# efirdc/Segmentation-Pipeline

Hardware: AMD Instinct MI355X
Metric: 3D patches/sec (128³, 4ch) train+infer at 1/2/4/8 MI355X; Dice vs CPU ref (higher is better)
Workload: dtype f32 (tensors, results and accumulation; the products of the 3x3x3 convolutions with >= 8 input channels run as six bf16 MFMAs on an EXACT three-way bf16 split of both f32 operands -- error vs f64 equal to the f32 MFMA kernels', profiles/r04_f32x3_accuracy.txt; the same step on v_mfma_f32_32x32x2_f32

## Files before the change

### include/m355seg.h

```cpp
#ifndef M355SEG_H
#define M355SEG_H

#include <stddef.h>
#include <stdint.h>

#ifdef __cplusplus
extern "C" {
#endif

#define M355_ABI_VERSION 3

enum {
  M355_OK = 0,
  M355_EINVALID_ARG = -1,
  M355_EUNSUPPORTED = -2,
  M355_ELAUNCH = -3,
  M355_EWORKSPACE = -4
};

enum { M355_F32 = 0 };

enum { M355_COMPUTE_F32 = 0, M355_COMPUTE_BF16 = 1, M355_COMPUTE_F16 = 2, M355_COMPUTE_F32X3 = 3 };

enum { M355_ACT_NONE = 0, M355_ACT_RELU = 1, M355_ACT_LEAKY_RELU = 2, M355_ACT_ELU = 3, M355_ACT_GELU = 4,
// ... 68 lines not shown

int m355_conv3d_launch_plan(int32_t entry, const m355_conv3d_desc* d, const int64_t* batch_strides, const uint64_t* pointers,
                            size_t workspace_bytes, int64_t* out12);

size_t m355_conv3d_bwd_data_workspace(const m355_conv3d_desc* d);
int m355_conv3d_bwd_data(const m355_conv3d_desc* d, const float* dy, const float* w,
                         float* dx, void* workspace, size_t workspace_bytes, void* stream);

size_t m355_conv3d_bwd_weight_workspace(const m355_conv3d_desc* d);
int m355_conv3d_bwd_weight(const m355_conv3d_desc* d, const float* x, const float* dy,
                           float* dw, float* dbias,
                           void* workspace, size_t workspace_bytes, void* stream);

size_t m355_conv_transpose3d_workspace(const m355_conv3d_desc* d);
int m355_conv_transpose3d_fwd(const m355_conv3d_desc* d, const float* x, const float* w,
                              const float* bias, float* y,
                              void* workspace, size_t workspace_bytes, void* stream);
int m355_conv_transpose3d_bwd_data(const m355_conv3d_desc* d, const float* dy, const float* w,
                                   float* dx, void* workspace, size_t workspace_bytes,
                                   void* stream);
int m355_conv_transpose3d_bwd_weight(const m355_conv3d_desc* d, const float* x, const float* dy,
                                     float* dw, float* dbias,
                                     void* workspace, size_t workspace_bytes, void* stream);

int m355_conv_transpose3d_plan(const m355_conv3d_desc* d, int32_t which, const void* y_side, int32_t* out4);

int32_t m355_conv_transpose3d_x3_bwd_supported(const m355_conv3d_desc* d, const void* y_side);
size_t m355_conv_transpose3d_x3_bwd_workspace(const m355_conv3d_desc* d);
int m355_conv_transpose3d_x3_bwd_plan(const m355_conv3d_desc* d, int32_t which, const void* y_side, int32_t* out4);
int m355_conv_transpose3d_bwd_data_x3(const m355_conv3d_desc* d, const float* dy, const float* w, float* dx,
                                      void* workspace, size_t workspace_bytes, void* stream);
int m355_conv_transpose3d_bwd_weight_x3(const m355_conv3d_desc* d, const float* x, const float* dy, float* dw, float* dbias,
                                        void* workspace, size_t workspace_bytes, void* stream);

int m355_conv_transpose3d_fwd_h16(const m355_conv3d_desc* d, const void* x16, int64_t x16_batch_stride,
                                  const float* w, const float* bias, void* y16, int64_t y16_batch_stride,
                                  int32_t compute, void* stream);

typedef struct m355_norm_desc {
  int32_t N, C;
  int64_t S;
  int32_t groups;
  int32_t act;
  float eps;
  float act_slope;
  int64_t x_batch_stride;
  int64_t y_batch_stride;
  int64_t add_batch_stride;
} m355_norm_desc;

int64_t m355_norm_num_stats(const m355_norm_desc* d);
size_t m355_norm_workspace(const m355_norm_desc* d);

int m355_norm_plan(const m355_norm_desc* d, int32_t which, int32_t* out4);

int m355_norm_stats(const m355_norm_desc* d, const float* x, float* mean, float* rstd,
                    float* running_mean, float* running_var, float momentum,
                    void* workspace, size_t workspace_bytes, void* stream);
int m355_norm_stats_from_partials(const m355_norm_desc* d, const float* stat_partials, int64_t slots,
                                  float* mean, float* rstd, float* running_mean, float* running_var,
                                  float momentum, void* workspace, size_t workspace_bytes, void* stream);
int m355_norm_stats_from_running(const m355_norm_desc* d, const float* running_mean,
                                 const float* running_var, float* mean, float* rstd,
                                 void* stream);
int m355_norm_act_fwd(const m355_norm_desc* d, const float* x, const float* mean,
                      const float* rstd, const float* gamma, const float* beta,
// ... 526 lines not shown
```

### segmentation-pipeline_amd/_lib.py

```python
import ctypes as C
import os

_HERE = os.path.dirname(os.path.abspath(__file__))
LIB_PATH = os.environ.get("M355_LIB_PATH") or os.path.join(_HERE, "libm355seg.so")

M355_OK = 0
M355_EUNSUPPORTED = -2
ACT_NONE, ACT_RELU, ACT_LEAKY_RELU = 0, 1, 2
ACT_ELU, ACT_GELU, ACT_GELU_TANH, ACT_SILU = 3, 4, 5, 6
COMPUTE_F32, COMPUTE_BF16, COMPUTE_F16, COMPUTE_F32X3 = 0, 1, 2, 3
CONV_W_PACKED, CONV_SOFTMAX, CONV_SIGMOID = 1, 2, 4


class ConvDesc(C.Structure):
    _fields_ = [
        ("N", C.c_int32), ("Cin", C.c_int32), ("Cout", C.c_int32),
        ("D", C.c_int32), ("H", C.c_int32), ("W", C.c_int32),
        ("k", C.c_int32), ("stride", C.c_int32), ("pad", C.c_int32), ("out_pad", C.c_int32),
        ("x_batch_stride", C.c_int64), ("y_batch_stride", C.c_int64),
        ("compute", C.c_int32), ("flags", C.c_int32),
    ]


class PackItem(C.Structure):
# ... 156 lines not shown
    "m355_norm_act_bwd_c8": (C.c_int, [_ND, _P, _i64, _P, _i64, _P, _i64, _i32, _i32, _i32, _P, _P, _P, _P, _P, _i64, _P, _P,
                                       C.c_int, _f32, _i32, _P, _sz, _P]),
    "m355_norm_act_bwd_c8_reduce": (C.c_int, [_ND, _P, _i64, _P, _i64, _P, _i64, _i32, _i32, _i32, _P, _P, _P, _P, _P, _P,
                                              C.c_int, _P, _f32, _P, _i32, _P, _sz, _P]),
    "m355_norm_act_bwd_c8_apply": (C.c_int, [_ND, _P, _i64, _P, _i64, _P, _i64, _i32, _i32, _i32, _P, _P, _P, _P, _P, _P, _i64,
                                             _i32, _P]),
    "m355_avgpool3d_2x_bwd_h16": (C.c_int, [_P, _P, _P, _i32, _i32, _i32, _i32, _i32, _i64, _i64, _i64, _i32, _P]),
    "m355_upsample_trilinear2x_fwd_h16": (C.c_int, [_P, _P, _i32, _i32, _i32, _i32, _i32, _i64, _i64, _i32, _P]),
    "m355_upsample_trilinear2x_bwd_h16": (C.c_int, [_P, _P, _i32, _i32, _i32, _i32, _i32, _i64, _i64, _i32, _P]),
    "m355_act16_channel_scale": (C.c_int, [_P, _P, _P, _i32, _i32, _i64, _i64, _i64, _i32, _P]),
    "m355_space_to_depth2_h16": (C.c_int, [_P, _P, _i32, _i32, _i32, _i32, _i32, _i64, _i64, _i32, _P]),
    "m355_depth_to_space2_h16": (C.c_int, [_P, _P, _i32, _i32, _i32, _i32, _i32, _i64, _i64, _i32, _P]),
    "m355_conv_transpose3d_h16_bwd_supported": (_i32, [_CD]),
    "m355_conv_transpose3d_h16_bwd_workspace": (_sz, [_CD]),
    "m355_conv_transpose3d_bwd_data_h16": (C.c_int, [_CD, _P, _i64, _P, _P, _i64, _i32, _P]),
    "m355_conv_transpose3d_bwd_weight_h16": (C.c_int, [_CD, _P, _i64, _P, _i64, _P, _P, _f32, _i32, _P, _sz, _P]),
    "m355_conv3d_plan": (C.c_int, [_CD, _i32, C.POINTER(C.c_int32)]),
    "m355_conv3d_launch_plan": (C.c_int, [_i32, _CD, C.POINTER(_i64), C.POINTER(C.c_uint64), _sz, C.POINTER(_i64)]),
    "m355_conv3d_bwd_data_workspace": (_sz, [_CD]),
    "m355_conv3d_bwd_data": (C.c_int, [_CD, _P, _P, _P, _P, _sz, _P]),
    "m355_conv3d_bwd_weight_workspace": (_sz, [_CD]),
    "m355_conv3d_bwd_weight": (C.c_int, [_CD, _P, _P, _P, _P, _P, _sz, _P]),
    "m355_conv_transpose3d_workspace": (_sz, [_CD]),
    "m355_conv_transpose3d_plan": (C.c_int, [_CD, _i32, _P, C.POINTER(C.c_int32)]),
    "m355_conv_transpose3d_fwd": (C.c_int, [_CD, _P, _P, _P, _P, _P, _sz, _P]),
    "m355_conv_transpose3d_bwd_data": (C.c_int, [_CD, _P, _P, _P, _P, _sz, _P]),
    "m355_conv_transpose3d_bwd_weight": (C.c_int, [_CD, _P, _P, _P, _P, _P, _sz, _P]),
    "m355_conv_transpose3d_fwd_h16": (C.c_int, [_CD, _P, _i64, _P, _P, _P, _i64, _i32, _P]),
    "m355_conv_transpose3d_x3_bwd_supported": (_i32, [_CD, _P]),
    "m355_conv_transpose3d_x3_bwd_workspace": (_sz, [_CD]),
    "m355_conv_transpose3d_x3_bwd_plan": (C.c_int, [_CD, _i32, _P, C.POINTER(C.c_int32)]),
    "m355_conv_transpose3d_bwd_data_x3": (C.c_int, [_CD, _P, _P, _P, _P, _sz, _P]),
    "m355_conv_transpose3d_bwd_weight_x3": (C.c_int, [_CD, _P, _P, _P, _P, _P, _sz, _P]),
    "m355_norm_num_stats": (_i64, [_ND]),
    "m355_norm_workspace": (_sz, [_ND]),
    "m355_norm_plan": (C.c_int, [_ND, _i32, C.POINTER(C.c_int32)]),
    "m355_norm_stats": (C.c_int, [_ND, _P, _P, _P, _P, _P, _f32, _P, _sz, _P]),
    "m355_norm_stats_from_partials": (C.c_int, [_ND, _P, _i64, _P, _P, _P, _P, _f32, _P, _sz, _P]),
    "m355_norm_stats_from_running": (C.c_int, [_ND, _P, _P, _P, _P, _P]),
    "m355_norm_act_fwd": (C.c_int, [_ND, _P, _P, _P, _P, _P, _P, _P, _P]),
    "m355_norm_act_pool_fwd": (C.c_int, [_ND, _P, _P, _P, _P, _P, _P, _P, _i64, _i32, _i32, _i32, _P]),
    "m355_norm_act_bwd": (C.c_int, [_ND, _P, _P, _P, _P, _P, _P, _P, _P, _P, C.c_int, _P, _sz, _P]),
    "m355_norm_act_bwd_pool": (C.c_int, [_ND, _P, _P, _i64, _P, _i64, _i32, _i32, _i32, _P, _P, _P, _P, _P, _P, _P, C.c_int,
                                         _P, _sz, _P]),
    "m355_norm_sums": (C.c_int, [_ND, _P, _P, _i64, _P, _P, _sz, _P]),
    "m355_norm_stats_from_sums": (C.c_int, [_ND, _P, _P, _P, _P, _P, _f32, _P]),
    "m355_norm_act_bwd_reduce": (C.c_int, [_ND, _P, _P, _P, _P, _P, _P, _P, _P, C.c_int, _P, _P, _P, _sz, _P]),
    "m355_norm_act_bwd_apply": (C.c_int, [_ND, _P, _P, _P, _P, _P, _P, _P, _P, _P, _i64, _i32, _P]),
    "m355_norm_act_bwd_h16": (C.c_int, [_ND, _P, _P, _P, _P, _P, _P, _P, _P, _P, C.c_int, _P, _i64, _i32, _P, _sz, _P]),
    "m355_resample_plan": (C.c_int, [_i32, _i32, _i32, _i32, _i32, _i32, C.POINTER(_i64), C.POINTER(C.c_uint64), _i32,
                                     C.POINTER(_i64)]),
    "m355_avgpool3d_2x_fwd": (C.c_int, [_P, _P, _i32, _i32, _i32, _i32, _i32, _i64, _i64, _P]),
    "m355_avgpool3d_2x_bwd": (C.c_int, [_P, _P, _i32, _i32, _i32, _i32, _i32, _i64, _i64, _P]),
    "m355_avgpool3d_2x_bwd_add": (C.c_int, [_P, _P, _P, _i32, _i32, _i32, _i32, _i32, _i64, _i64, _i64, _P]),
    "m355_maxpool3d_2x_fwd": (C.c_int, [_P, _P, _P, _i32, _i32, _i32, _i32, _i32, _i64, _i64, _P]),
    "m355_maxpool3d_2x_bwd": (C.c_int, [_P, _P, _P, _P, _i32, _i32, _i32, _i32, _i32, _i64, _i64, _i64, _P]),
    "m355_maxpool3d_2x_fwd_h16": (C.c_int, [_P, _P, _P, _i32, _i32, _i32, _i32, _i32, _i64, _i64, _i32, _P]),
    "m355_maxpool3d_2x_bwd_h16": (C.c_int, [_P, _P, _P, _P, _i32, _i32, _i32, _i32, _i32, _i64, _i64, _i64, _i32, _P]),
    "m355_upsample_trilinear2x_fwd": (C.c_int, [_P, _P, _i32, _i32, _i32, _i32, _i32, _i64, _i64, _P]),
    "m355_upsample_trilinear2x_bwd": (C.c_int, [_P, _P, _i32, _i32, _i32, _i32, _i32, _i64, _i64, _P]),
    "m355_upsample_nearest2x_fwd": (C.c_int, [_P, _P, _i32, _i32, _i32, _i32, _i32, _i64, _i64, _P]),
    "m355_upsample_nearest2x_bwd": (C.c_int, [_P, _P, _i32, _i32, _i32, _i32, _i32, _i64, _i64, _P]),
    "m355_upsample_trilinear2x_hp_fwd": (C.c_int, [_P, _P, _i32, _i32, _i32, _i32, _i32, _i64, _i64, _P]),
    "m355_upsample_trilinear2x_hp_bwd": (C.c_int, [_P, _P, _i32, _i32, _i32, _i32, _i32, _i64, _i64, _P]),
    "m355_upsample_nearest2x_fwd_h16": (C.c_int, [_P, _P, _i32, _i32, _i32, _i32, _i32, _i64, _i64, _i32, _P]),
    "m355_upsample_nearest2x_bwd_h16": (C.c_int, [_P, _P, _i32, _i32, _i32, _i32, _i32, _i64, _i64, _i32, _P]),
# ... 215 lines not shown
```

### segmentation-pipeline_amd/csrc/abi.cpp

```cpp
#include "common.hpp"
#include <map>
#include <mutex>
#include <tuple>
#include <utility>

namespace m355 {
static thread_local char g_err[512] = "";
void set_error(const char* fmt, ...) {
  va_list ap;
  va_start(ap, fmt);
  vsnprintf(g_err, sizeof(g_err), fmt, ap);
  va_end(ap);
}

static int env_int(const char* name, int dflt) {
  const char* v = getenv(name);
  if (!v || !*v) return dflt;
  return atoi(v);
}
static Tuning read_tuning() {
  Tuning t;
  t.conv_ntw = env_int("M355_CONV_NTW", 0);
  t.conv_ksplit = env_int("M355_CONV_KSPLIT", 0);
  t.conv_slots = env_int("M355_CONV_SLOTS", 0);
  t.conv_persistent = env_int("M355_CONV_PERSISTENT", 1);
  t.no_small = env_int("M355_NO_SMALL", 0);
  t.smallcout_valu = env_int("M355_SMALLCOUT_VALU", 1);
  t.f32x3 = env_int("M355_F32X3", 1);
  t.f32x3_bww = env_int("M355_F32X3_BWW", 1);
  t.f32x3_edge = env_int("M355_F32X3_EDGE", 0);
  t.f32x3_convt = env_int("M355_F32X3_CONVT", 1);
  t.f32x3_convt_bwd = env_int("M355_F32X3_CONVT_BWD", 1);
  t.bww_nsplit = env_int("M355_BWW_NSPLIT", 0);
  t.bww_gen = env_int("M355_BWW_GEN", 2);
  t.bww_queue = env_int("M355_BWW_QUEUE", 1);
  t.h16_persistent = env_int("M355_H16_PERSISTENT", 1);
  t.tile16 = env_int("M355_TILE16", 1);
  t.convt_h16 = env_int("M355_CONVT_H16", 1);
  t.h16_w8 = env_int("M355_H16_W8", 1);
  t.h16_oneshot = env_int("M355_H16_ONESHOT", 1);
  t.h16_xcd = env_int("M355_H16_XCD", 1);
  t.conv_cube = env_int("M355_CONV_CUBE", 3);
  t.h16_order = env_int("M355_H16_ORDER", 3);
  t.fuse_softmax = env_int("M355_FUSE_SOFTMAX", 1);
  t.convt_wgs = env_int("M355_CONVT_WGS", 0);
  t.h16_stagger = env_int("M355_H16_STAGGER", 2);
  return t;
}
static Tuning g_tuning = read_tuning();
const Tuning& tuning() { return g_tuning; }

int num_cus() {
  static int cache[64] = {0};
  int dev = 0;
  if (hipGetDevice(&dev) != hipSuccess || dev < 0 || dev >= 64) {
    (void)hipGetLastError();
    return 256;
  }
  if (cache[dev] == 0) {
    int n = 0;
    if (hipDeviceGetAttribute(&n, hipDeviceAttributeMultiprocessorCount, dev) != hipSuccess || n <= 0) {
      (void)hipGetLastError();
      n = 256;
    }
    cache[dev] = n;
// ... 86 lines not shown
```

### segmentation-pipeline_amd/csrc/common.hpp

```cpp
#pragma once
#include <hip/hip_runtime.h>
#include <stdint.h>
#include <stdio.h>
#include <stdarg.h>
#include <stdlib.h>
#include <algorithm>
#include "../../include/m355seg.h"

namespace m355 {

void set_error(const char* fmt, ...);

static inline int64_t ceil_div(int64_t a, int64_t b) { return (a + b - 1) / b; }
static inline int64_t round_up(int64_t a, int64_t b) { return ceil_div(a, b) * b; }

static inline int check_launch(const char* what) {
  hipError_t e = hipGetLastError();
  if (e != hipSuccess) {
    set_error("%s: launch failed: %s", what, hipGetErrorString(e));
    return M355_ELAUNCH;
  }
  return M355_OK;
}

// ... 24 lines not shown
    const uint32_t o = (uint32_t)__shfl_up((int)v, off, 64);
    if (lane >= off) v += o;
  }
  return v;
}

template <typename T, int NT, bool BCAST = false>
__device__ __forceinline__ T block_sum(T v, T* scratch) {
  v = wave_sum(v);
  const int lane = threadIdx.x & 63, w = threadIdx.x >> 6;
  __syncthreads();
  if (lane == 0) scratch[w] = v;
  __syncthreads();
  T r = T(0);
  if (BCAST || threadIdx.x == 0) {
#pragma unroll
    for (int i = 0; i < NT / 64; ++i) r += scratch[i];
  }
  return r;
}

__device__ __forceinline__ float sigmoid_f32(float v) { return 1.f / (1.f + expf(-v)); }

struct Tuning {
  int conv_ntw = 0, conv_ksplit = 0, conv_slots = 0, conv_persistent = 1;
  int no_small = 0, smallcout_valu = 1, bww_nsplit = 0, bww_gen = 2, bww_queue = 1, h16_persistent = 1, tile16 = 1, convt_h16 = 1, h16_w8 = 1, h16_oneshot = 1, h16_xcd = 1;
  int conv_cube = 3, h16_order = 3;
  int fuse_softmax = 1;
  int f32x3 = 1;
  int f32x3_bww = 1;
  int f32x3_edge = 0;
  int f32x3_convt = 1;
  int f32x3_convt_bwd = 1;
  int convt_wgs = 0;
  int h16_stagger = 2;
};
const Tuning& tuning();

static inline int64_t dense_or(int64_t stride, int64_t dense) { return stride ? stride : dense; }

int num_cus();

int* queue_state(hipStream_t st);
int* overflow_flag();

}
```

### segmentation-pipeline_amd/csrc/conv3d_common.hpp

```cpp
#pragma once
#include "common.hpp"
#include "h16.hpp"
#include "conv3d_route.hpp"

namespace m355 {


__device__ __forceinline__ int opaque(int v) {
  asm volatile("" : "+v"(v));
  return v;
}

__device__ __forceinline__ void queue_leave(int* __restrict__ counter) {
  if (threadIdx.x == 0) {
    if (atomicAdd(counter + 8, 1) == (int)gridDim.x - 1) {
#pragma unroll
      for (int r = 0; r < 9; ++r) counter[r] = 0;
    }
  }
}

template <int NTW, int GX>
struct FwdTile {
  static constexpr int GY = 32 / GX;
// ... 122 lines not shown
        }
      }
      if (ok) {
#pragma unroll
        for (int r = 0; r < 4; ++r)
          if (ob + r < Cout) dst[base + (int64_t)r * DHW] = v[r];
      }
    }
  if (stat) {
#pragma unroll
    for (int r = 0; r < 4; ++r) {
#pragma unroll
      for (int off = 8; off >= 1; off >>= 1) {
        s1[r] += __shfl_xor(s1[r], off, 64);
        s2[r] += __shfl_xor(s2[r], off, 64);
      }
    }
    if ((lane & 15) == 0) {
#pragma unroll
      for (int r = 0; r < 4; ++r)
        if (ob + r < Cout) {
          stat[(int64_t)(ob + r) * 2] = s1[r];
          stat[(int64_t)(ob + r) * 2 + 1] = s2[r];
        }
    }
  }
}

int convt_fwd_x3_nvt(int Cin);
void launch_convt_fwd_x3(int nvt, dim3 grid, const float* x, const float* w, const float* bias, float* y, int Cin, int Cout,
                         int D, int H, int W, int64_t xbs, int64_t ybs, int mt_per_wg, hipStream_t st);
void launch_convt_bww_x3(int mt, dim3 grid, const float* x, const float* dy, float* dw, float* dbias, float* slab, double* bslab,
                         int N, int Cin, int Cout, int D, int H, int W, int64_t xbs, int64_t ybs, hipStream_t st);

enum class ConvtKind {
  Direct,
  MfmaF32,
  X3,
  C8,
  H16,
  Unsupported
};
struct ConvtRoute {
  ConvtKind kind;
  int nvt;
  int mt;
  int mt_per_wg;
  int ks_n, ng;
  dim3 grid;
  size_t lds;
  int split, o_per_split;
  size_t slab_bytes;
  size_t dbias_offset, dbias_bytes;
  size_t workspace_bytes;
  int32_t plan_code[4];
};
ConvtRoute route_convt(const m355_conv3d_desc* d, int which, bool y_side_ok);
ConvtRoute route_convt_c8(const m355_conv3d_desc* d, int which);

struct ConvCall {
  const m355_conv3d_desc* d;
  const float* in;
  const void* in16;
  const float* w;
  const float* bias;
  const float* add;
// ... 86 lines not shown
```

### segmentation-pipeline_amd/csrc/conv3d_f32x3.hip

```cpp
#include "conv3d_common.hpp"

namespace m355 {

typedef __bf16 bf16x8 __attribute__((ext_vector_type(8)));
typedef unsigned u32x4 __attribute__((ext_vector_type(4)));

constexpr int X3_PAIRS = 14;
constexpr int X3_QUADS = 7;
__host__ __device__ constexpr int x3_pair_tap(int pair, int half) {
  return pair < 9 ? pair * 3 + half : (pair < 12 ? (pair - 9) * 9 + half * 3 + 2 : (pair == 12 ? half * 9 + 8 : 26));
}

__device__ __forceinline__ void x3_split(float v, unsigned& hi, unsigned& mid, unsigned& lo) {
  const unsigned u = __float_as_uint(v);
  hi = u & 0xffff0000u;
  const float r1 = (u & 0x7f800000u) == 0x7f800000u ? 0.f : v - __uint_as_float(hi);
  mid = __float_as_uint(r1) & 0xffff0000u;
  lo = __float_as_uint(r1 - __uint_as_float(mid));
}
__device__ __forceinline__ unsigned x3_pack(unsigned a, unsigned b) { return __builtin_amdgcn_perm(b, a, 0x07060302u); }

__device__ __forceinline__ void pack_w3_x3_item(const float* __restrict__ w, u32x4* __restrict__ wq, int64_t i, int Cout_w,
                                                int Cin_w, int kin, int mout, int nchunks, int transpose) {
  const int lane = (int)(i & 63);
// ... 1222 lines not shown
  const int64_t i = (int64_t)(bias ? blockIdx.x - eblocks : blockIdx.x) * 32 + e;
  double v = 0.0;
  if (i < n) {
    if (bias) {
      for (int s = q; s < nsplit; s += 8) v += bslab[(int64_t)s * n + i];
    } else {
#pragma unroll 4
      for (int s = q; s < nsplit; s += 8) v += (double)slab[(int64_t)s * n + i];
    }
  }
  red[q][e] = v;
  __syncthreads();
  if (q == 0 && i < n) {
    const double r = ((red[0][e] + red[1][e]) + (red[2][e] + red[3][e])) + ((red[4][e] + red[5][e]) + (red[6][e] + red[7][e]));
    (bias ? dbias : out)[i] = (float)r;
  }
}

void launch_convt_bww_x3(int mt, dim3 grid, const float* x, const float* dy, float* dw, float* dbias, float* slab, double* bslab,
                         int N, int Cin, int Cout, int D, int H, int W, int64_t xbs, int64_t ybs, hipStream_t st) {
  const int nsplit = (int)grid.x;
  if (mt == 2)
    hipLaunchKernelGGL(convt_k2s2_bwd_weight_x3_kernel<2>, grid, dim3(256), 0, st, x, dy, slab, bslab, N, Cin, Cout, D, H, W,
                       xbs, ybs, nsplit);
  else
    hipLaunchKernelGGL(convt_k2s2_bwd_weight_x3_kernel<4>, grid, dim3(256), 0, st, x, dy, slab, bslab, N, Cin, Cout, D, H, W,
                       xbs, ybs, nsplit);
  const int64_t total = (int64_t)Cin * Cout * 8;
  const int eblocks = (int)ceil_div(total, 32), bblocks = dbias ? (int)ceil_div(Cout, 32) : 0;
  hipLaunchKernelGGL(convt_k2s2_slab_reduce_x3_kernel, dim3((unsigned)(eblocks + bblocks)), dim3(256), 0, st, slab, dw, total,
                     nsplit, bslab, dbias, Cout, eblocks);
}

}
```

### segmentation-pipeline_amd/csrc/conv3d_host.hip

```cpp
#include "conv3d_common.hpp"

using namespace m355;

static ConvRoute query_conv(const m355_conv3d_desc* d, int which) { return route_conv(d, conv_query_args(which)); }
static BwwRoute query_bww(const m355_conv3d_desc* d) { return route_bww(d, conv_query_args(2)); }
static BwwRoute query_bww_c8(const m355_conv3d_desc* d) {
  ConvArgs a{};
  a.entry = CE_BWD_WEIGHT_H16;
  return route_bww_c8(d, a);
}

extern "C" size_t m355_conv3d_fwd_workspace(const m355_conv3d_desc* d) { return d ? query_conv(d, 0).workspace_bytes : 0; }
extern "C" size_t m355_conv3d_bwd_data_workspace(const m355_conv3d_desc* d) { return d ? query_conv(d, 1).workspace_bytes : 0; }
extern "C" size_t m355_conv3d_h16_workspace(const m355_conv3d_desc* d, int32_t which) {
  return d ? query_conv(d, which).h16_workspace_bytes : 0;
}
extern "C" size_t m355_conv3d_bwd_weight_workspace(const m355_conv3d_desc* d) { return d ? query_bww(d).workspace_bytes : 0; }
extern "C" size_t m355_conv3d_bwd_weight_h16_workspace(const m355_conv3d_desc* d) {
  return d ? query_bww_c8(d).h16_workspace_bytes : 0;
}
extern "C" size_t m355_conv3d_bwd_weight_c8_workspace(const m355_conv3d_desc* d) {
  return d ? query_bww_c8(d).c8_workspace_bytes : 0;
}
extern "C" size_t m355_conv3d_packed_bytes(const m355_conv3d_desc* d, int32_t which) {
// ... 157 lines not shown

extern "C" int m355_conv3d_bwd_data_h16_c8(const m355_conv3d_desc* d, const void* dy16, int64_t dy16_batch_stride,
                                           const float* w, void* dx16, int64_t dx16_batch_stride, void* workspace,
                                           size_t workspace_bytes, void* stream) {
  return run_conv({CE_BWD_DATA_H16_C8, P(dy16), P(w), 0, 0, P(dx16), 0, P(workspace), workspace_bytes,
                   {dy16_batch_stride, dx16_batch_stride}}, d, stream);
}

static int run_bww(const ConvArgs& a, const m355_conv3d_desc* d, float grad_unscale, void* stream) {
  BwwRoute r;
  if (int rc = check_bww(a, d, &r)) return rc;
  const BwwCall c = {d, (const void*)a.in, (const void*)a.w, (const float*)(a.entry == CE_BWD_WEIGHT ? a.w : a.bias),
                     (float*)a.out, (float*)a.stat, grad_unscale, (void*)a.ws, (hipStream_t)stream};
  return launch_bww(r, c);
}

extern "C" int m355_conv3d_bwd_weight(const m355_conv3d_desc* d, const float* x, const float* dy, float* dw, float* dbias,
                                      void* workspace, size_t workspace_bytes, void* stream) {
  return run_bww({CE_BWD_WEIGHT, P(x), P(dy), 0, 0, P(dw), P(dbias), P(workspace), workspace_bytes, {0, 0}}, d, 1.f, stream);
}

extern "C" int m355_conv3d_bwd_weight_h16(const m355_conv3d_desc* d, const void* x16, int64_t x16_batch_stride,
                                          const void* dy16, int64_t dy16_batch_stride, const float* dy, float* dw,
                                          float* dbias, void* workspace, size_t workspace_bytes, void* stream) {
  return run_bww({CE_BWD_WEIGHT_H16, P(x16), P(dy16), P(dy), 0, P(dw), P(dbias), P(workspace), workspace_bytes,
                  {x16_batch_stride, dy16_batch_stride}}, d, 1.f, stream);
}

extern "C" int m355_conv3d_bwd_weight_c8(const m355_conv3d_desc* d, const void* x16, int64_t x16_batch_stride,
                                         const void* dy16, int64_t dy16_batch_stride, float* dw, float* dbias,
                                         float grad_unscale, void* workspace, size_t workspace_bytes, void* stream) {
  return run_bww({CE_BWD_WEIGHT_C8, P(x16), P(dy16), 0, 0, P(dw), P(dbias), P(workspace), workspace_bytes,
                  {x16_batch_stride, dy16_batch_stride}}, d, grad_unscale, stream);
}

extern "C" int m355_conv3d_launch_plan(int32_t entry, const m355_conv3d_desc* d, const int64_t* batch_strides,
                                       const uint64_t* pointers, size_t workspace_bytes, int64_t* out12) {
  M355_REQUIRE(entry >= 0 && entry < CE_COUNT && batch_strides && pointers && out12, M355_EINVALID_ARG,
               "conv3d_launch_plan: bad entry point index / null pointer");
  const ConvArgs a = {entry, (uintptr_t)pointers[0], (uintptr_t)pointers[1], (uintptr_t)pointers[2], (uintptr_t)pointers[3],
                      (uintptr_t)pointers[4], (uintptr_t)pointers[5], (uintptr_t)pointers[6], workspace_bytes,
                      {batch_strides[0], batch_strides[1]}};
  if (entry == CE_BWD_WEIGHT || entry == CE_BWD_WEIGHT_H16 || entry == CE_BWD_WEIGHT_C8) {
    BwwRoute r;
    if (int rc = check_bww(a, d, &r)) return rc;
    const int64_t o[12] = {(int64_t)r.kind, r.grid.x, r.grid.y, r.grid.z, r.block, 0, 0, r.aux, (int64_t)r.need, r.reduce_grid.x,
                           (int64_t)r.dbias_off, (int64_t)r.x16_off};
    std::copy_n(o, 12, out12);
  } else {
    ConvRoute r;
    if (int rc = check_conv(a, d, &r)) return rc;
    const int64_t o[12] = {(int64_t)r.kind, r.grid.x, r.grid.y, r.grid.z, r.block, r.grid16.x, r.grid16.z, r.aux, (int64_t)r.need,
                           r.reduce_grid.x, (int64_t)r.slab_off, (int64_t)r.stage_off};
    std::copy_n(o, 12, out12);
  }
  return M355_OK;
}
```

### segmentation-pipeline_amd/csrc/conv3d_route.hpp

```cpp
#pragma once
#include "h16.hpp"

namespace m355 {

inline bool is16(int compute) { return compute == M355_COMPUTE_BF16 || compute == M355_COMPUTE_F16; }
inline int out_dim(int in, int k, int s, int p) { return (in + 2 * p - k) / s + 1; }
inline int64_t splitk_c8_slots(int64_t S) { return std::max<int64_t>(1, std::min<int64_t>(ceil_div(S, 256), 2048)); }
constexpr int SMALLCOUT_TZ_K = 90, SMALLCOUT_VS_TZ = 4, SMALLCOUT_VS_TY = 8, SMALLCOUT_VS_TX = 64;
inline size_t smallcout_packed_bytes(int Cin) { return (size_t)round_up((int64_t)round_up(Cin, 2) * SMALLCOUT_TZ_K * 32 * 4, 256); }

struct FwdPlan {
  bool mfma;
  bool persistent;
  int gx, ntw;
  int tz_tiles, ty_tiles, tx_tiles;
  int otiles, kin_pad, mout_pad, nchunks, ksplit;
  int tile16;
  int nw;
  int oneshot;
  int x3;
  int64_t slots;
  size_t wp_bytes, slab_bytes;
};
struct BwwClasses {
// ... 795 lines not shown
  const char* who = CONV_ENTRY_NAMES[a.entry];
  if (int rc = validate_conv(d, who)) return rc;
  const int64_t S = (int64_t)d->D * d->H * d->W;
  if (a.entry == CE_BWD_WEIGHT) {
    M355_REQUIRE(a.in && a.w && a.out, M355_EINVALID_ARG, "conv3d_bwd_weight: null pointer");
    const BwwRoute& r = *route = route_bww(d, a);
    M355_REQUIRE(a.ws && a.ws_bytes >= r.need, M355_EWORKSPACE, "conv3d_bwd_weight: workspace too small (%zu < %zu)",
                 a.ws_bytes, r.need);
    M355_REQUIRE(r.kind == BwwKind::Direct || r.kind == BwwKind::X3 || r.kind == BwwKind::X3c ||
                     ((int64_t)d->Cin * S < (1ll << 31) && (int64_t)d->Cout * S < (1ll << 31)),
                 M355_EUNSUPPORTED, "conv3d_bwd_weight: tensor exceeds 2^31 elements per sample");
    if (r.via_pack)
      M355_REQUIRE((a.ws & 15) == 0, M355_EINVALID_ARG, "conv3d_bwd_weight_h16: c8 tensor not 16B aligned");
    else if (r.kind == BwwKind::Direct)
      M355_REQUIRE((int64_t)d->Cout * d->Cin * d->k * d->k * d->k < (1ll << 31), M355_EUNSUPPORTED,
                   "conv3d_bwd_weight: grid too large");
    else if (r.kind == BwwKind::X3 || r.kind == BwwKind::X3c)
      M355_REQUIRE(((a.in | a.w) & 3) == 0, M355_EINVALID_ARG, "conv3d_bwd_weight: misaligned tensor");
    return M355_OK;
  }
  const bool c8_flow = a.entry == CE_BWD_WEIGHT_C8;
  const BwwRoute& r = *route = route_bww_c8(d, a);
  M355_REQUIRE(r.h16, M355_EUNSUPPORTED,
               "%s: c8 input is only defined for the 3x3x3 / stride 1 / pad 1 kernels in a 16-bit compute mode", who);
  M355_REQUIRE(a.in && a.w && a.out && a.ws, M355_EINVALID_ARG, "%s: null pointer", who);
  M355_REQUIRE(r.ok, M355_EUNSUPPORTED, "%s: volume too large for the c8 kernel (>= 2^25 voxels)", who);
  M355_REQUIRE(c8_flow || !a.stat || a.bias, M355_EINVALID_ARG, "%s: the bias gradient needs the fp32 dy", who);
  M355_REQUIRE(a.ws_bytes >= r.need, M355_EWORKSPACE, "%s: workspace too small (%zu < %zu)", who, a.ws_bytes, r.need);
  M355_REQUIRE(((a.in | a.w) & 15) == 0 && r.xbs % 8 == 0 && r.ybs % 8 == 0, M355_EINVALID_ARG,
               "%s: c8 tensor not 16B aligned", who);
  return M355_OK;
}

}
```

### segmentation-pipeline_amd/ops.py

```python
import ctypes as C
import math
import os
import weakref
from dataclasses import dataclass
from operator import itemgetter
from typing import List, NamedTuple, Optional, Sequence

import numpy as np
import torch

from . import _lib
from ._lib import ACT_LEAKY_RELU, ACT_NONE, ACT_RELU, ConvDesc, NormDesc, check

FP32_SPLIT = os.environ.get("M355_FP32_SPLIT", "1") != "0"
_COMPUTE = {"fp32": _lib.COMPUTE_F32X3 if FP32_SPLIT else _lib.COMPUTE_F32, "fp32_mfma": _lib.COMPUTE_F32,
            "bf16": _lib.COMPUTE_BF16, "fp16": _lib.COMPUTE_F16}
_DT16 = {_lib.COMPUTE_BF16: torch.bfloat16, _lib.COMPUTE_F16: torch.float16}
_compute_mode = "fp32"


def set_precision(mode: str):
    global _compute_mode
    if mode not in _COMPUTE:
        raise ValueError(f"precision must be one of {sorted(_COMPUTE)}, not {mode!r}")
# ... 384 lines not shown
    if w is None:
        return None
    d = _deferred.get(idx)
    if d is None:
        d = _deferred[idx] = _DeferredOverflow()
        d.host = torch.zeros(1, dtype=torch.int32).pin_memory()
        d.event = torch.cuda.Event()
    elif d.armed and d.event.query():
        _adapt_after_overflow(int(d.host[0]))
        d.armed = False
    found = (w != 0).to(torch.float32).reshape(())
    if not d.armed:
        d.host.copy_(w, non_blocking=True)
        d.event.record()
        d.armed = True
    w.zero_()
    return found


def fp16_overflow(device=None) -> int:
    hit = 0
    for idx, w in _overflow_words.items():
        if device is not None and device.index not in (None, idx):
            continue
        v = int(w.item())
        if v:
            w.zero_()
            hit |= v
    _adapt_after_overflow(hit)
    return hit
FUSE_POOL = os.environ.get("M355_FUSE_POOL", "1") != "0"
FUSE_POOL_BWD = os.environ.get("M355_FUSE_POOL_BWD", "1") != "0"
fused_bwd_counts = {"pool": 0}


_pack_registry = {}
PACK_BATCH = os.environ.get("M355_PACK_BATCH", "1") != "0"
_pack_scope = None


class pack_scope:
    def __init__(self, params):
        self.ids = {id(p) for p in params}
        self.params = list(params)

    def __enter__(self):
        global _pack_scope
        self.prev, _pack_scope = _pack_scope, self.ids
        for p in self.params:
            cache = getattr(p, "_m355_packed", None)
            if cache is not None:
                p._m355_packed = (-1, cache[1], cache[2])
        return self

    def __exit__(self, *exc):
        global _pack_scope
        _pack_scope = self.prev


def _repack_stale(L, device):
    items = []
    for key, ref in list(_pack_registry.items()):
        if _pack_scope is not None and key not in _pack_scope:
            continue
        w = ref()
        cache = getattr(w, "_m355_packed", None) if w is not None else None
# ... 559 lines not shown
        L = _lib.lib()
        meta = ctx.meta
        d = ctx.desc
        if meta.softmax or meta.sigmoid:
            x, weight, y = ctx.saved_tensors
            dy = _head_bwd(y, dy, meta.softmax)
        else:
            x, weight = ctx.saved_tensors
        dy, dybs = _dense_channels(dy)
        if dybs != d.y_batch_stride:
            d = _conv_desc(d.N, d.Cin, d.Cout, d.D, d.H, d.W, d.k, d.stride, d.pad, d.x_batch_stride, dybs, compute=d.compute)
        need_w, need_b, need_add = ctx.needs_input_grad[0], ctx.needs_input_grad[1], ctx.needs_input_grad[2]
        need_x = any(ctx.needs_input_grad[4:])
        dw = db = dadd = None
        dparts: List[Optional[torch.Tensor]] = [None] * len(ctx.part_channels)
        x16 = dy16 = None
        if ctx.x16 is not None:
            x16 = Act16(x, *ctx.x16)
            x_dtype, x_device = ctx.x_meta
            dy16 = _c8_twin(dy, x16.compute)
            if dy16 is None:
                dy16 = pack_act16(dy, x16.compute)
        else:
            x_dtype, x_device = x.dtype, x.device
        if need_w or (need_b and ctx.has_bias):
            dw = torch.empty_like(weight)
            db = torch.empty(d.Cout, dtype=weight.dtype, device=weight.device) if ctx.has_bias else None
            if x16 is not None:
                ws = _workspace(L.m355_conv3d_bwd_weight_h16_workspace(C.byref(d)), x_device)
                _conv_launch("conv3d_bwd_weight", d, None, 4, 4, L.m355_conv3d_bwd_weight_h16, C.byref(d), x16.ptr(),
                             x16.batch_stride(), dy16.ptr(), dy16.batch_stride(), _p(dy) if db is not None else None,
                             _p(dw), _p(db), _p(ws), ws.numel(), _stream())
            else:
                ws = _workspace(L.m355_conv3d_bwd_weight_workspace(C.byref(d)), x_device)
                _conv_launch("conv3d_bwd_weight", d, 2, 4, 4, L.m355_conv3d_bwd_weight, C.byref(d), _p(x), _p(dy),
                             _p(dw), _p(db), _p(ws), ws.numel(), _stream())
        if need_x:
            dx = torch.empty((d.N, d.Cin, d.D, d.H, d.W), dtype=x_dtype, device=x_device)
            dd = _conv_desc(d.N, d.Cin, d.Cout, d.D, d.H, d.W, d.k, d.stride, d.pad, 0, d.y_batch_stride, compute=d.compute)
            wbuf, flags = _packed_weight(weight, dd, 1)
            ddk = _with_flags(dd, flags)
            if dy16 is not None:
                ws = _workspace(L.m355_conv3d_h16_workspace(C.byref(dd), 1), x_device)
                _conv_launch("conv3d_bwd_data", dd, 1, 4, 4, L.m355_conv3d_bwd_data_h16, C.byref(ddk), dy16.ptr(),
                             dy16.batch_stride(), _p(wbuf), _p(dx), _p(ws), ws.numel(), _stream())
            else:
                ws = _workspace(L.m355_conv3d_bwd_data_workspace(C.byref(dd)), x_device)
                _conv_launch("conv3d_bwd_data", dd, 1, 4, 4, L.m355_conv3d_bwd_data, C.byref(ddk), _p(dy), _p(wbuf),
                             _p(dx), _p(ws), ws.numel(), _stream())
            c0 = 0
            for i, cc in enumerate(ctx.part_channels):
                if ctx.needs_input_grad[4 + i]:
                    dparts[i] = dx if len(ctx.part_channels) == 1 else dx[:, c0:c0 + cc]
                c0 += cc
        if need_add and ctx.has_add:
            dadd = dy
        return (dw if need_w else None, db if need_b else None, dadd, None, *dparts)


def conv3d(x, weight, bias=None, add=None, stride=1, padding=1, out: Optional[OutSlot] = None,
           stats: Optional[dict] = None, c8_out: bool = False, softmax: bool = False, sigmoid: bool = False):
    if softmax and sigmoid:
        raise ValueError("conv3d: softmax and sigmoid exclude each other (one hypothesis head per output convolution)")
    head = softmax or sigmoid
    k = weight.shape[2]
    if not (weight.shape[2] == weight.shape[3] == weight.shape[4]):
        raise NotImplementedError("only cubic kernels are supported")
    c8_parts = None
    if isinstance(x, Concat) and isinstance(x.buf, Act16):
# ... 1921 lines not shown
```

Measured before the change: 48.67.

## Add split-bf16 MFMA weight-gradient kernel for edge convs with few channels

Adds a dedicated backward-weight kernel for 3x3x3 convolutions with at most 4 channels on one side (the input and output edge layers) in F32X3 mode. The f32 operands are split three ways into bf16 in LDS, each of the 27 taps is mapped to a lane group, and the product runs as bf16 MFMAs with double-buffered register staging. Partial results from many tile splits go to a slab that a separate kernel reduces in double precision. The Python path tries this route first and falls back to the generic bwd_weight, at the cost of an extra reduction launch and more workspace.

```diff
diff --git a/include/m355seg.h b/include/m355seg.h
--- a/include/m355seg.h
+++ b/include/m355seg.h
@@ -124,6 +124,12 @@
                                       void* workspace, size_t workspace_bytes, void* stream);
 int m355_conv_transpose3d_bwd_weight_x3(const m355_conv3d_desc* d, const float* x, const float* dy, float* dw, float* dbias,
                                         void* workspace, size_t workspace_bytes, void* stream);
+
+int32_t m355_conv3d_bwd_weight_x3_edge_supported(const m355_conv3d_desc* d, const void* x, const void* dy);
+size_t m355_conv3d_bwd_weight_x3_edge_workspace(const m355_conv3d_desc* d);
+int m355_conv3d_bwd_weight_x3_edge_plan(const m355_conv3d_desc* d, const void* x, const void* dy, int32_t* out4);
+int m355_conv3d_bwd_weight_x3_edge(const m355_conv3d_desc* d, const float* x, const float* dy, float* dw, float* dbias,
+                                   void* workspace, size_t workspace_bytes, void* stream);
 
 int m355_conv_transpose3d_fwd_h16(const m355_conv3d_desc* d, const void* x16, int64_t x16_batch_stride,
                                   const float* w, const float* bias, void* y16, int64_t y16_batch_stride,
diff --git a/segmentation-pipeline_amd/_lib.py b/segmentation-pipeline_amd/_lib.py
--- a/segmentation-pipeline_amd/_lib.py
+++ b/segmentation-pipeline_amd/_lib.py
@@ -212,6 +212,10 @@
     "m355_conv_transpose3d_x3_bwd_plan": (C.c_int, [_CD, _i32, _P, C.POINTER(C.c_int32)]),
     "m355_conv_transpose3d_bwd_data_x3": (C.c_int, [_CD, _P, _P, _P, _P, _sz, _P]),
     "m355_conv_transpose3d_bwd_weight_x3": (C.c_int, [_CD, _P, _P, _P, _P, _P, _sz, _P]),
+    "m355_conv3d_bwd_weight_x3_edge_supported": (_i32, [_CD, _P, _P]),
+    "m355_conv3d_bwd_weight_x3_edge_workspace": (_sz, [_CD]),
+    "m355_conv3d_bwd_weight_x3_edge_plan": (C.c_int, [_CD, _P, _P, C.POINTER(C.c_int32)]),
+    "m355_conv3d_bwd_weight_x3_edge": (C.c_int, [_CD, _P, _P, _P, _P, _P, _sz, _P]),
     "m355_norm_num_stats": (_i64, [_ND]),
     "m355_norm_workspace": (_sz, [_ND]),
     "m355_norm_plan": (C.c_int, [_ND, _i32, C.POINTER(C.c_int32)]),
diff --git a/segmentation-pipeline_amd/csrc/abi.cpp b/segmentation-pipeline_amd/csrc/abi.cpp
--- a/segmentation-pipeline_amd/csrc/abi.cpp
+++ b/segmentation-pipeline_amd/csrc/abi.cpp
@@ -31,6 +31,8 @@
   t.f32x3_edge = env_int("M355_F32X3_EDGE", 0);
   t.f32x3_convt = env_int("M355_F32X3_CONVT", 1);
   t.f32x3_convt_bwd = env_int("M355_F32X3_CONVT_BWD", 1);
+  t.f32x3_edge_bww = env_int("M355_F32X3_EDGE_BWW", 1);
+  t.edge_bww_nsplit = env_int("M355_EDGE_BWW_NSPLIT", 0);
   t.bww_nsplit = env_int("M355_BWW_NSPLIT", 0);
   t.bww_gen = env_int("M355_BWW_GEN", 2);
   t.bww_queue = env_int("M355_BWW_QUEUE", 1);
diff --git a/segmentation-pipeline_amd/csrc/common.hpp b/segmentation-pipeline_amd/csrc/common.hpp
--- a/segmentation-pipeline_amd/csrc/common.hpp
+++ b/segmentation-pipeline_amd/csrc/common.hpp
@@ -80,6 +80,8 @@
   int f32x3_edge = 0;
   int f32x3_convt = 1;
   int f32x3_convt_bwd = 1;
+  int f32x3_edge_bww = 1;
+  int edge_bww_nsplit = 0;
   int convt_wgs = 0;
   int h16_stagger = 2;
 };
diff --git a/segmentation-pipeline_amd/csrc/conv3d_common.hpp b/segmentation-pipeline_amd/csrc/conv3d_common.hpp
--- a/segmentation-pipeline_amd/csrc/conv3d_common.hpp
+++ b/segmentation-pipeline_amd/csrc/conv3d_common.hpp
@@ -178,6 +178,9 @@
                          int D, int H, int W, int64_t xbs, int64_t ybs, int mt_per_wg, hipStream_t st);
 void launch_convt_bww_x3(int mt, dim3 grid, const float* x, const float* dy, float* dw, float* dbias, float* slab, double* bslab,
                          int N, int Cin, int Cout, int D, int H, int W, int64_t xbs, int64_t ybs, hipStream_t st);
+
+void launch_edge_bww_x3(dim3 grid, const float* x, const float* dy, float* dw, float* slab, const m355_conv3d_desc* d,
+                        int tz_tiles, int ty_tiles, int tx_tiles, int64_t xbs, int64_t ybs, hipStream_t st);
 
 enum class ConvtKind {
   Direct,
diff --git a/segmentation-pipeline_amd/csrc/conv3d_f32x3.hip b/segmentation-pipeline_amd/csrc/conv3d_f32x3.hip
--- a/segmentation-pipeline_amd/csrc/conv3d_f32x3.hip
+++ b/segmentation-pipeline_amd/csrc/conv3d_f32x3.hip
@@ -1278,4 +1278,223 @@
                      nsplit, bslab, dbias, Cout, eblocks);
 }
 
-}
+struct EdgeTile {
+  static constexpr int TX = 32, TY = 2, TZ = 2, QZS = 336, QXS = 1360, QCS = 4160;
+  __device__ static constexpr unsigned long long taps(int wave) {
+    return wave == 0 ? 0x9e58a4863a20ull : wave == 1 ? 0xb6b9aaa71c2eull : wave == 2 ? 0xcefb32df9db4ull : 0x035e80600038ull;
+  }
+};
+
+__global__ __launch_bounds__(256, 2) void conv3_edge_bww_x3_kernel(
+    const float* __restrict__ P, const float* __restrict__ Q, float* __restrict__ slab, int N, int CP, int CQ, int D, int H,
+    int W, int tz_tiles, int ty_tiles, int tx_tiles, int nsplit, int64_t pbs, int64_t qbs, int swap, int Cin, int Cout) {
+  using T = EdgeTile;
+  constexpr int TX = T::TX, TY = T::TY, TZ = T::TZ, NV = TX * TY * TZ;
+  static_assert(NV == 128, "64 voxel pairs: one per lane of a staging wave");
+  constexpr int PRS = NV * 2 + 16, PPL = 32 * PRS;
+  constexpr int QRS = TX * 2 + 16, QZS = T::QZS, QXS = T::QXS, QCS = T::QCS, QPL = 4 * QCS;
+  constexpr int HY = TY + 2, HR = (TZ + 2) * HY, QW = TX / 2, QPER = 4 * HR * QW / 256, XK = TX / 16;
+  static_assert(4 * HR * QW % 256 == 0 && QZS >= HY * QRS && QXS >= (TZ + 2) * QZS && QCS >= 3 * QXS, "narrow planes");
+  constexpr unsigned OOB = 0x80000000u;
+  __shared__ __attribute__((aligned(16))) unsigned char ps3[3 * PPL];
+  __shared__ __attribute__((aligned(16))) unsigned char qs3[3 * QPL];
+
+  const int tid = threadIdx.x, lane = tid & 63;
+  const int wave = __builtin_amdgcn_readfirstlane(tid >> 6);
+  const int half = lane >> 5, l32 = lane & 31;
+  const int p0 = blockIdx.x * 32, split = blockIdx.y;
+  const int iHW = H * W, iDHW = D * H * W;
+
+  const int s_l = l32 & 3, t8 = l32 >> 2;
+  const unsigned tcode = (unsigned)(T::taps(wave) >> (6 * t8)) & 63u;
+  const int tap_eff = (int)(tcode & 31u);
+  const bool tap_ok = (tcode >> 5) != 0;
+  const unsigned char* qb = qs3 + s_l * QCS + (tap_eff % 3) * QXS + (tap_eff / 9) * QZS + ((tap_eff / 3) % 3) * QRS + half * 16;
+  const unsigned char* pb = ps3 + l32 * PRS + half * 16;
+
+  f32x16 acc0, acc1;
+#pragma unroll
+  for (int r = 0; r < 16; ++r) acc0[r] = acc1[r] = 0.f;
+
+  const int tiles_per_n = tz_tiles * ty_tiles * tx_tiles;
+  const int ntiles = N * tiles_per_n;
+
+  const int prow = (2 * lane) / TX, px = (2 * lane) % TX, pz = prow / TY, py = prow % TY;
+  unsigned qrel[QPER], qlds[QPER], qcode[QPER];
+#pragma unroll
+  for (int k = 0; k < QPER; ++k) {
+    const int e = tid + 256 * k;
+    const int c = e / (HR * QW), r = e - c * (HR * QW);
+    const int hr = r / QW, xw = r - hr * QW;
+    const int zz = hr / HY, yy = hr - zz * HY;
+    qrel[k] = (unsigned)c * (unsigned)iDHW + (unsigned)(zz * iHW + yy * W + 2 * xw);
+    qlds[k] = (unsigned)(c * QCS + zz * QZS + yy * QRS + xw * 4);
+    qcode[k] = c < CQ ? ((unsigned)zz | ((unsigned)yy << 8) | ((unsigned)(2 * xw) << 16)) : 0xFFu;
+  }
+
+  struct Stage {
+    float2 pr[8];
+    float qr[QPER][4];
+  };
+  auto fetch = [&](Stage& s, int tile) __attribute__((always_inline)) {
+    const bool live = tile < ntiles;
+    int t = live ? tile : 0;
+    const int n = t / tiles_per_n;
+    t -= n * tiles_per_n;
+    const int txt = t % tx_tiles;
+    t /= tx_tiles;
+    const int tyt = t % ty_tiles;
+    const int tzt = t / ty_tiles;
+    const int z0 = tzt * TZ, y0 = tyt * TY, x0 = txt * TX;
+    const __amdgpu_buffer_rsrc_t rp =
+        __builtin_amdgcn_make_buffer_rsrc((void*)(P + (int64_t)n * pbs), 0, live ? CP * iDHW * 4 : 0, 0x00020000);
+    const __amdgpu_buffer_rsrc_t rq =
+        __builtin_amdgcn_make_buffer_rsrc((void*)(Q + (int64_t)n * qbs), 0, live ? CQ * iDHW * 4 : 0, 0x00020000);
+    const int gz = z0 + pz, gy = y0 + py, gx = x0 + px;
+    const bool vok = gz < D && gy < H && gx < W;
+    const unsigned sp = (unsigned)(p0 + wave) * (unsigned)iDHW + (unsigned)(gz * iHW + gy * W + gx);
+#pragma unroll
+    for (int j = 0; j < 8; ++j) {
+      const bool ok = vok && p0 + wave + 4 * j < CP;
+      s.pr[j] = __builtin_bit_cast(
+          float2, __builtin_amdgcn_raw_buffer_load_b64(rp, ok ? (sp + (unsigned)(4 * j) * (unsigned)iDHW) * 4u : OOB, 0, 0));
+    }
+    const int qbase = (z0 - 1) * iHW + (y0 - 1) * W + (x0 - 1);
+#pragma unroll
+    for (int k = 0; k < QPER; ++k) {
+      const unsigned cd = qcode[k];
+      const bool rok = (unsigned)(z0 - 1 + (int)(cd & 0xFFu)) < (unsigned)D && (unsigned)(y0 - 1 + (int)((cd >> 8) & 0xFFu)) < (unsigned)H;
+      const int xq = x0 - 1 + (int)(cd >> 16);
+#pragma unroll
+      for (int m = 0; m < 4; ++m) {
+        const bool ok = rok && (unsigned)(xq + m) < (unsigned)W;
+        s.qr[k][m] = __builtin_bit_cast(
+            float, __builtin_amdgcn_raw_buffer_load_b32(rq, ok ? ((unsigned)qbase + qrel[k] + (unsigned)m) * 4u : OOB, 0, 0));
+      }
+    }
+  };
+  auto commit = [&](const Stage& s) __attribute__((always_inline)) {
+#pragma unroll
+    for (int j = 0; j < 8; ++j) {
+      unsigned ha, ma, la, hb, mb, lb;
+      x3_split(s.pr[j].x, ha, ma, la);
+      x3_split(s.pr[j].y, hb, mb, lb);
+      unsigned char* row = ps3 + (wave + 4 * j) * PRS + lane * 4;
+      *reinterpret_cast<unsigned*>(row) = x3_pack(ha, hb);
+      *reinterpret_cast<unsigned*>(row + PPL) = x3_pack(ma, mb);
+      *reinterpret_cast<unsigned*>(row + 2 * PPL) = x3_pack(la, lb);
+    }
+#pragma unroll
+    for (int k = 0; k < QPER; ++k) {
+      unsigned h[4], m[4], l[4];
+#pragma unroll
+      for (int i = 0; i < 4; ++i) x3_split(s.qr[k][i], h[i], m[i], l[i]);
+      unsigned char* w0 = qs3 + qlds[k];
+#pragma unroll
+      for (int dx = 0; dx < 3; ++dx) {
+        *reinterpret_cast<unsigned*>(w0 + dx * QXS) = x3_pack(h[dx], h[dx + 1]);
+        *reinterpret_cast<unsigned*>(w0 + dx * QXS + QPL) = x3_pack(m[dx], m[dx + 1]);
+        *reinterpret_cast<unsigned*>(w0 + dx * QXS + 2 * QPL) = x3_pack(l[dx], l[dx + 1]);
+      }
+    }
+  };
+
+  auto multiply = [&]() __attribute__((always_inline)) {
+#pragma unroll
+    for (int ks = 0; ks < NV / 16; ks += 2) {
+      bf16x8 ah[2], am[2], al[2], bh[2], bm[2], bl[2];
+#pragma unroll
+      for (int u = 0; u < 2; ++u) {
+        const int row = (ks + u) / XK, xh = (ks + u) % XK;
+        const unsigned char* a = pb + (ks + u) * 32;
+        const unsigned char* b = qb + (row / TY) * QZS + (row % TY) * QRS + xh * 32;
+        ah[u] = *reinterpret_cast<const bf16x8*>(a);
+        am[u] = *reinterpret_cast<const bf16x8*>(a + PPL);
+        al[u] = *reinterpret_cast<const bf16x8*>(a + 2 * PPL);
+        bh[u] = *reinterpret_cast<const bf16x8*>(b);
+        bm[u] = *reinterpret_cast<const bf16x8*>(b + QPL);
+        bl[u] = *reinterpret_cast<const bf16x8*>(b + 2 * QPL);
+      }
+      acc0 = __builtin_amdgcn_mfma_f32_32x32x16_bf16(al[0], bh[0], acc0, 0, 0, 0);
+      acc1 = __builtin_amdgcn_mfma_f32_32x32x16_bf16(al[1], bh[1], acc1, 0, 0, 0);
+      acc0 = __builtin_amdgcn_mfma_f32_32x32x16_bf16(am[0], bh[0], acc0, 0, 0, 0);
+      acc1 = __builtin_amdgcn_mfma_f32_32x32x16_bf16(am[1], bh[1], acc1, 0, 0, 0);
+      acc0 = __builtin_amdgcn_mfma_f32_32x32x16_bf16(ah[0], bh[0], acc0, 0, 0, 0);
+      acc1 = __builtin_amdgcn_mfma_f32_32x32x16_bf16(ah[1], bh[1], acc1, 0, 0, 0);
+      acc0 = __builtin_amdgcn_mfma_f32_32x32x16_bf16(am[0], bm[0], acc0, 0, 0, 0);
+      acc1 = __builtin_amdgcn_mfma_f32_32x32x16_bf16(am[1], bm[1], acc1, 0, 0, 0);
+      acc0 = __builtin_amdgcn_mfma_f32_32x32x16_bf16(ah[0], bm[0], acc0, 0, 0, 0);
+      acc1 = __builtin_amdgcn_mfma_f32_32x32x16_bf16(ah[1], bm[1], acc1, 0, 0, 0);
+      acc0 = __builtin_amdgcn_mfma_f32_32x32x16_bf16(ah[0], bl[0], acc0, 0, 0, 0);
+      acc1 = __builtin_amdgcn_mfma_f32_32x32x16_bf16(ah[1], bl[1], acc1, 0, 0, 0);
+    }
+  };
+
+  Stage sa, sb;
+  fetch(sa, split);
+  fetch(sb, split + nsplit);
+  for (int tile = split; tile < ntiles; tile += 2 * nsplit) {
+    __syncthreads();
+    commit(sa);
+    __syncthreads();
+    fetch(sa, tile + 2 * nsplit);
+    multiply();
+    if (tile + nsplit < ntiles) {
+      __syncthreads();
+      commit(sb);
+      __syncthreads();
+      fetch(sb, tile + 3 * nsplit);
+      multiply();
+    }
+  }
+  if (tap_ok && s_l < CQ) {
+    float* sl = slab + (int64_t)split * Cout * Cin * 27;
+    const int tap = swap ? 26 - tap_eff : tap_eff;
+#pragma unroll
+    for (int r = 0; r < 16; ++r) {
+      const int i = p0 + (r & 3) + 8 * (r >> 2) + 4 * half;
+      if (i < CP) {
+        const int o = swap ? s_l : i, c = swap ? i : s_l;
+        sl[((int64_t)o * Cin + c) * 27 + tap] = acc0[r] + acc1[r];
+      }
+    }
+  }
+}
+
+__global__ __launch_bounds__(256) void conv3_edge_slab_reduce_x3_kernel(const float* __restrict__ slab, float* __restrict__ out,
+                                                                        int total, int nsplit) {
+  __shared__ double red[16][17];
+  const int e = threadIdx.x & 15, q = threadIdx.x >> 4;
+  const int i = (int)blockIdx.x * 16 + e;
+  double v = 0.0;
+  if (i < total) {
+#pragma unroll 8
+    for (int s = q; s < nsplit; s += 16) v += (double)slab[(int64_t)s * total + i];
+  }
+  red[q][e] = v;
+  __syncthreads();
+  if (q == 0 && i < total) {
+    double t[16];
+#pragma unroll
+    for (int k = 0; k < 16; ++k) t[k] = red[k][e];
+#pragma unroll
+    for (int w = 1; w < 16; w *= 2)
+#pragma unroll
+      for (int k = 0; k < 16; k += 2 * w) t[k] += t[k + w];
+    out[i] = (float)t[0];
+  }
+}
+
+void launch_edge_bww_x3(dim3 grid, const float* x, const float* dy, float* dw, float* slab, const m355_conv3d_desc* d,
+                        int tz_tiles, int ty_tiles, int tx_tiles, int64_t xbs, int64_t ybs, hipStream_t st) {
+  const int swap = d->Cin <= 4 ? 0 : 1, nsplit = (int)grid.y;
+  const float *P = swap ? x : dy, *Q = swap ? dy : x;
+  const int CP = swap ? d->Cin : d->Cout, CQ = swap ? d->Cout : d->Cin;
+  hipLaunchKernelGGL(conv3_edge_bww_x3_kernel, grid, dim3(256), 0, st, P, Q, slab, d->N, CP, CQ, d->D, d->H, d->W, tz_tiles,
+                     ty_tiles, tx_tiles, nsplit, swap ? xbs : ybs, swap ? ybs : xbs, swap, d->Cin, d->Cout);
+  const int total = d->Cout * d->Cin * 27;
+  hipLaunchKernelGGL(conv3_edge_slab_reduce_x3_kernel, dim3((unsigned)ceil_div(total, 16)), dim3(256), 0, st, slab, dw, total,
+                     nsplit);
+}
+
+}
diff --git a/segmentation-pipeline_amd/csrc/conv3d_host.hip b/segmentation-pipeline_amd/csrc/conv3d_host.hip
--- a/segmentation-pipeline_amd/csrc/conv3d_host.hip
+++ b/segmentation-pipeline_amd/csrc/conv3d_host.hip
@@ -213,6 +213,41 @@
                                          float grad_unscale, void* workspace, size_t workspace_bytes, void* stream) {
   return run_bww({CE_BWD_WEIGHT_C8, P(x16), P(dy16), 0, 0, P(dw), P(dbias), P(workspace), workspace_bytes,
                   {x16_batch_stride, dy16_batch_stride}}, d, grad_unscale, stream);
+}
+
+extern "C" int32_t m355_conv3d_bwd_weight_x3_edge_supported(const m355_conv3d_desc* d, const void* x, const void* dy) {
+  return d && route_edge_bww_x3(d, x, dy).ok ? 1 : 0;
+}
+extern "C" size_t m355_conv3d_bwd_weight_x3_edge_workspace(const m355_conv3d_desc* d) {
+  return d ? route_edge_bww_x3(d, nullptr, nullptr).workspace_bytes : 0;
+}
+extern "C" int m355_conv3d_bwd_weight_x3_edge_plan(const m355_conv3d_desc* d, const void* x, const void* dy, int32_t* out4) {
+  if (int rc = validate_conv(d, "conv3d_bwd_weight_x3_edge_plan")) return rc;
+  M355_REQUIRE(out4, M355_EINVALID_ARG, "conv3d_bwd_weight_x3_edge_plan: null pointer");
+  const EdgeBwwRoute r = route_edge_bww_x3(d, x, dy);
+  std::copy_n(r.plan_code, 4, out4);
+  return M355_OK;
+}
+extern "C" int m355_conv3d_bwd_weight_x3_edge(const m355_conv3d_desc* d, const float* x, const float* dy, float* dw, float* dbias,
+                                              void* workspace, size_t workspace_bytes, void* stream) {
+  const char* who = "conv3d_bwd_weight_x3_edge";
+  if (int rc = validate_conv(d, who)) return rc;
+  M355_REQUIRE(x && dy && dw, M355_EINVALID_ARG, "%s: null pointer", who);
+  const EdgeBwwRoute r = route_edge_bww_x3(d, x, dy);
+  M355_REQUIRE(r.ok, M355_EUNSUPPORTED,
+               "%s: needs M355_COMPUTE_F32X3, kernel_size 3 / stride 1 / padding 1, at most 4 channels on one side, even W, the "
+               "wide tensor 8-byte aligned with an even batch stride and below 2^29 elements per sample, at least 2^21 voxels "
+               "in the batch, and M355_F32X3 / M355_F32X3_EDGE_BWW not 0 (m355_conv3d_bwd_weight_x3_edge_supported): take "
+               "m355_conv3d_bwd_weight", who);
+  const size_t need = dbias ? r.workspace_bytes : r.slab_bytes;
+  M355_REQUIRE(workspace && workspace_bytes >= need, M355_EWORKSPACE, "%s: workspace too small (%zu < %zu)", who,
+               workspace_bytes, need);
+  M355_REQUIRE(((uintptr_t)workspace & 15) == 0 && (((uintptr_t)x | (uintptr_t)dy | (uintptr_t)dw) & 3) == 0, M355_EINVALID_ARG,
+               "%s: misaligned tensor or workspace", who);
+  hipStream_t st = (hipStream_t)stream;
+  launch_edge_bww_x3(r.grid, x, dy, dw, (float*)workspace, d, r.tz_tiles, r.ty_tiles, r.tx_tiles, r.xbs, r.ybs, st);
+  if (dbias) launch_dbias(dy, dbias, d->N, d->Cout, out_voxels(d), r.ybs, (char*)workspace + r.dbias_off, st);
+  return check_launch(who);
 }
 
 extern "C" int m355_conv3d_launch_plan(int32_t entry, const m355_conv3d_desc* d, const int64_t* batch_strides,
diff --git a/segmentation-pipeline_amd/csrc/conv3d_route.hpp b/segmentation-pipeline_amd/csrc/conv3d_route.hpp
--- a/segmentation-pipeline_amd/csrc/conv3d_route.hpp
+++ b/segmentation-pipeline_amd/csrc/conv3d_route.hpp
@@ -851,4 +851,46 @@
   return M355_OK;
 }
 
-}
+constexpr int64_t EDGE_X3_BWW_MIN_VOXELS = 1ll << 21;
+struct EdgeBwwRoute {
+  bool ok;
+  int nsplit, swap;
+  int tz_tiles, ty_tiles, tx_tiles;
+  dim3 grid;
+  int64_t xbs, ybs;
+  size_t slab_bytes, dbias_off, workspace_bytes;
+  int32_t plan_code[4];
+};
+static inline EdgeBwwRoute route_edge_bww_x3(const m355_conv3d_desc* d, const void* x, const void* dy) {
+  EdgeBwwRoute r{};
+  const int knob = tuning().f32x3_edge_bww;
+  if (d->N <= 0 || d->Cin <= 0 || d->Cout <= 0 || d->D <= 0 || d->H <= 0 || d->W <= 0) return r;
+  if (d->compute != M355_COMPUTE_F32X3 || !tuning().f32x3 || !knob || !is_k3s1p1(d)) return r;
+  if (std::min(d->Cin, d->Cout) > 4) return r;
+  const int64_t S = (int64_t)d->D * d->H * d->W;
+  r.swap = d->Cin <= 4 ? 0 : 1;
+  r.xbs = dense_or(d->x_batch_stride, (int64_t)d->Cin * S);
+  r.ybs = dense_or(d->y_batch_stride, (int64_t)d->Cout * S);
+  const int wide = r.swap ? d->Cin : d->Cout;
+  const int64_t wide_bs = r.swap ? r.xbs : r.ybs;
+  const void* wide_ptr = r.swap ? x : dy;
+  if (d->W % 2 || wide_bs % 2 || ((uintptr_t)wide_ptr & 7) || (int64_t)wide * S >= (1ll << 29)) return r;
+  if (d->N * S < EDGE_X3_BWW_MIN_VOXELS && knob < 2) return r;
+  const int tx = 32, ty = 2, tz = 2;
+  r.tz_tiles = (int)ceil_div(d->D, tz);
+  r.ty_tiles = (int)ceil_div(d->H, ty);
+  r.tx_tiles = (int)ceil_div(d->W, tx);
+  const int64_t ntiles = (int64_t)d->N * r.tz_tiles * r.ty_tiles * r.tx_tiles;
+  if (ntiles >= (1ll << 30)) return r;
+  const int64_t ptiles = ceil_div(wide, 32);
+  r.nsplit = (int)std::min(std::max<int64_t>(1, 2 * (int64_t)num_cus() / ptiles), ntiles);
+  if (tuning().edge_bww_nsplit > 0) r.nsplit = std::min(tuning().edge_bww_nsplit, 65535);
+  r.grid = dim3((unsigned)ptiles, (unsigned)r.nsplit);
+  r.slab_bytes = r.dbias_off = (size_t)round_up((int64_t)r.nsplit * d->Cout * d->Cin * 27 * 4, 256);
+  r.workspace_bytes = r.slab_bytes + dbias_ws_bytes(d->Cout, S);
+  r.ok = true;
+  r.plan_code[0] = 12; r.plan_code[1] = tx; r.plan_code[2] = r.nsplit; r.plan_code[3] = r.swap;
+  return r;
+}
+
+}
diff --git a/segmentation-pipeline_amd/ops.py b/segmentation-pipeline_amd/ops.py
--- a/segmentation-pipeline_amd/ops.py
+++ b/segmentation-pipeline_amd/ops.py
@@ -440,6 +440,21 @@
 FUSE_POOL = os.environ.get("M355_FUSE_POOL", "1") != "0"
 FUSE_POOL_BWD = os.environ.get("M355_FUSE_POOL_BWD", "1") != "0"
 fused_bwd_counts = {"pool": 0}
+edge_bww_counts = {"x3": 0}
+
+
+def m355_conv3d_bwd_weight(d, x, dy, dw, db, device):
+    L = _lib.lib()
+    if d.compute == _lib.COMPUTE_F32X3 and min(d.Cin, d.Cout) <= 4 and \
+            L.m355_conv3d_bwd_weight_x3_edge_supported(C.byref(d), _p(x), _p(dy)):
+        ws = _workspace(L.m355_conv3d_bwd_weight_x3_edge_workspace(C.byref(d)), device)
+        rc = L.m355_conv3d_bwd_weight_x3_edge(C.byref(d), _p(x), _p(dy), _p(dw), _p(db), _p(ws), ws.numel(), _stream())
+        if rc != _lib.M355_EUNSUPPORTED:
+            if rc == _lib.M355_OK:
+                edge_bww_counts["x3"] += 1
+            return rc
+    ws = _workspace(L.m355_conv3d_bwd_weight_workspace(C.byref(d)), device)
+    return L.m355_conv3d_bwd_weight(C.byref(d), _p(x), _p(dy), _p(dw), _p(db), _p(ws), ws.numel(), _stream())
 
 
 _pack_registry = {}
@@ -1065,9 +1080,7 @@
                              x16.batch_stride(), dy16.ptr(), dy16.batch_stride(), _p(dy) if db is not None else None,
                              _p(dw), _p(db), _p(ws), ws.numel(), _stream())
             else:
-                ws = _workspace(L.m355_conv3d_bwd_weight_workspace(C.byref(d)), x_device)
-                _conv_launch("conv3d_bwd_weight", d, 2, 4, 4, L.m355_conv3d_bwd_weight, C.byref(d), _p(x), _p(dy),
-                             _p(dw), _p(db), _p(ws), ws.numel(), _stream())
+                _conv_launch("conv3d_bwd_weight", d, 2, 4, 4, m355_conv3d_bwd_weight, d, x, dy, dw, db, x_device)
         if need_x:
             dx = torch.empty((d.N, d.Cin, d.D, d.H, d.W), dtype=x_dtype, device=x_device)
             dd = _conv_desc(d.N, d.Cin, d.Cout, d.D, d.H, d.W, d.k, d.stride, d.pad, 0, d.y_batch_stride, compute=d.compute)
```

Measured after the change: 48.98 (median of 6 runs). About the same (+0.6%).
